# michalfratczak/habdec

Measured on AMD Instinct MI355X. Metric: IQ Msamples/s (batched 2.048 MS/s streams), higher is better.
Workload: dtype f32

## Files before the change

habdec_amd/csrc/dev_types.h:

```cpp
#pragma once
#include <stdint.h>
#ifndef __HIPCC__
#ifndef __host__
#define __host__
#define __device__
#endif
#endif

namespace hd {

constexpr int kFftBins = 4096;
constexpr uint32_t kVentLimit = 30000;
constexpr uint32_t kFirBatch = 256;

struct StreamCall {
    uint32_t n_in;
    uint32_t n1;
    uint32_t n2;
    uint32_t zero_hist1;
    uint32_t zero_hist2;
    uint32_t pend_before;
    uint32_t fft_fill;
    uint32_t fft_take;
    uint32_t fft_run;
    uint32_t fir_m;
    uint32_t fir_taps;
    uint32_t fir_zero_hist;
    uint32_t pend_after;
    uint32_t dc_remove;
    uint32_t clear_pending;
    uint32_t fir_taps_prev;
};
__host__ __device__ inline uint32_t sc_taps_prev(const StreamCall& c) { return c.fir_taps_prev & 0xFFFFu; }
__host__ __device__ inline uint32_t sc_head_n(const StreamCall& c) { return (c.fir_taps_prev >> 16) & 0x3FFFu; }
__host__ __device__ inline bool sc_head_prev(const StreamCall& c) { return (c.fir_taps_prev >> 30) & 1u; }
__host__ __device__ inline bool sc_head_save(const StreamCall& c) { return (c.fir_taps_prev >> 31) & 1u; }
__host__ __device__ inline uint32_t sc_pack_taps_prev(uint32_t taps_prev, uint32_t head_n, bool head_prev, bool head_save)
{ return (taps_prev & 0xFFFFu) | ((head_n & 0x3FFFu) << 16) | ((head_prev ? 1u : 0u) << 30) | ((head_save ? 1u : 0u) << 31); }


struct SymbolParams {
    uint32_t spb;
    uint32_t R;
    uint32_t min_held;
    uint32_t float_abs;
    uint32_t reset;
};

struct SymState {
    uint32_t base;
    uint32_t held;
    uint32_t cached;
    uint32_t run_pos;
    float    run_sum;
    uint32_t _pad[3];
};

struct BitsHeader {
    uint32_t nbits;
    uint32_t held_after;
    uint32_t nflips;
    uint32_t overflow;
    uint32_t uncached;
    uint32_t demod_ck[2];
    uint32_t demod_n;
// ... 15 lines not shown
```

habdec_amd/csrc/engine.cpp:

```cpp
#include <hip/hip_runtime.h>
#include <rocfft/rocfft.h>

#include <algorithm>
#include <atomic>
#include <chrono>
#include <cmath>
#include <cstdio>
#include <cstdlib>
#include <cstring>
#include <memory>
#include <condition_variable>
#include <mutex>
#include <thread>
#include <string>
#include <vector>

#include "../../include/habdec_amd.h"
#include "dev_types.h"
#include "host/afc_tracker.hpp"
#include "host/decim_plan.hpp"
#include "host/fir_design.hpp"
#include "host/iq_file_batch.hpp"
#include "host/text_stage.hpp"
#include "kernels/launch.h"
// ... 17 lines not shown
    size_t n = 0;
    hipError_t alloc(size_t count)
    {
        n = count;
        hipError_t e = hipMalloc(reinterpret_cast<void**>(&p), std::max<size_t>(count, 1) * sizeof(T));
        if (e == hipSuccess) e = hipMemset(p, 0, std::max<size_t>(count, 1) * sizeof(T));
        return e;
    }
    ~DevBuf() { if (p) (void)hipFree(p); }
};
template <typename T>
struct PinBuf {
    T* p = nullptr;
    T* dev = nullptr;
    size_t n = 0;
    hipError_t alloc(size_t count)
    {
        n = count;
        hipError_t e = hipHostMalloc(reinterpret_cast<void**>(&p), std::max<size_t>(count, 1) * sizeof(T), hipHostMallocMapped | hipHostMallocCoherent);
        if (e == hipSuccess) std::memset(p, 0, std::max<size_t>(count, 1) * sizeof(T));
        if (e == hipSuccess) e = hipHostGetDevicePointer(reinterpret_cast<void**>(&dev), p, 0);
        return e;
    }
    ~PinBuf() { if (p) (void)hipHostFree(p); }
};

struct StreamHost {
    double baud = 300;
    float lp_bw = 1500, lp_trans = 0.025f;
    bool dc = false;
    size_t stage_buf[2] = {0, 0};
    size_t pending = 0;
    size_t fft_fill = 0;
    bool have_spectrum = false;
    uint64_t spectra = 0;
    size_t fir_buf = 0;
    uint32_t fir_T_run = 0;
    uint32_t head_n = 0;
    uint64_t head_call = ~0ull;
    bool head_aside = false;
    hd::LowpassDesigner lp;
    bool taps_dirty = false;
    uint32_t held = 0, win_ub = 0, inflight_m = 0;
    bool sym_reset = true;
    hd::TextStage text;
    hd::AfcTracker afc;
    hd::SpectrumStats stats{};
    uint32_t last_n2 = 0, last_pend_before = 0, last_m = 0, last_nbits = 0, last_nflips = 0;
    uint64_t flip_list_full = 0;
    uint64_t bits_total = 0;
    int last_buf = 0;
    std::vector<uint32_t> last_words;
    uint32_t demod_ck[2] = {0, 0}, demod_ck_n = 0xFFFFFFFFu;
    uint64_t demod_ck_call = 0;
    uint64_t demod_ck_hash = 0xCBF29CE484222325ull;
    uint64_t demod_ck_calls = 0, demod_ck_unknown = 0;
};

}

struct hd_engine {
    hd_engine_config cfg{};
    double fs = 0, fsd = 0;
    std::vector<hd::DecimStage> stages;
    uint32_t S = 0, D = 1;
    uint32_t n1_cap = 0, n2_cap = 0;
    uint32_t taps_cap = 0, fir_hist_cap = 0;
// ... 274 lines not shown
    } else
        e->no_claim = true;
    if (e->stages.size() >= 1) {
        for (auto& h : e->hist1) HD_HIP(h.alloc((size_t)S * (e->stages[0].taps.size() - 1)));
        HD_HIP(e->stage_taps[0].alloc(e->stages[0].taps.size() + 1));
        HD_HIP(hipMemcpy(e->stage_taps[0].p, e->stages[0].taps.data(), e->stages[0].taps.size() * 4, hipMemcpyHostToDevice));
    }
    if (e->stages.size() == 2) {
        for (auto& h : e->hist2) HD_HIP(h.alloc((size_t)S * (e->stages[1].taps.size() - 1)));
        HD_HIP(e->stage_taps[1].alloc(e->stages[1].taps.size() + 1));
        HD_HIP(hipMemcpy(e->stage_taps[1].p, e->stages[1].taps.data(), e->stages[1].taps.size() * 4, hipMemcpyHostToDevice));
    }
    for (auto& b : e->fbuf) HD_HIP(b.alloc((size_t)S * e->fbuf_stride));
    HD_HIP(e->lp_taps.alloc((size_t)S * e->taps_cap));
    HD_HIP(e->demod.alloc((size_t)S * m_cap));
    if (cfg->keep_filtered) HD_HIP(e->filtered.alloc((size_t)S * m_cap));
    HD_HIP(e->tail.alloc((size_t)S * e->tail_cap));
    HD_HIP(e->weight.alloc((size_t)S * e->tail_cap));
    HD_HIP(e->flipmask.alloc((size_t)S * (e->tail_cap / 64)));
    HD_HIP(e->d_symstate.alloc(S));
    if (e->flips_cap) HD_HIP(e->flips_dbg.alloc((size_t)S * e->flips_cap));
    for (auto& c : e->carry) HD_HIP(c.alloc(S));
    e->head_cap = std::min<uint32_t>(e->taps_cap, 8192u);
    HD_HIP(e->fir_head.alloc((size_t)S * e->head_cap));
    HD_HIP(e->demod_ck_acc.alloc((size_t)2 * S));
    HD_HIP(e->d_sym.alloc(S));
    HD_HIP(e->h_sym.alloc(S));
    for (auto& sl : e->slot) {
        HD_HIP(sl.d_call.alloc(S));
        HD_HIP(sl.h_call.alloc(S));
        HD_HIP(sl.h_slots.alloc((size_t)S * e->slot_words));
    }
    if (cfg->enable_spectrum) {
        HD_HIP(e->fft_in.alloc((size_t)S * hd::kFftBins));
        HD_HIP(e->fft_raw.alloc((size_t)S * hd::kFftBins));
        HD_HIP(e->spec.alloc((size_t)S * hd::kFftBins));
        HD_HIP(e->power.alloc((size_t)S * hd::kFftBins));
        for (auto& sl : e->slot) HD_HIP(sl.h_stats.alloc(S));
        {
            std::vector<float2> tw(hd::kFftBins);
            for (size_t m = 0; m < hd::kFftBins; ++m) {
                const double a = 2.0 * 3.14159265358979323846264338327950288 * (double)m / (double)hd::kFftBins;
                tw[m] = make_float2((float)std::cos(a), (float)-std::sin(a));
            }
            HD_HIP(e->fft_tw.alloc(hd::kFftBins));
            HD_HIP(hipMemcpy(e->fft_tw.p, tw.data(), tw.size() * sizeof(float2), hipMemcpyHostToDevice));
            e->tail_fft = getenv("HD_ROCFFT") == nullptr;
            e->own_fft = e->tail_fft || getenv("HD_OWN_FFT") != nullptr;
        }
        std::call_once(g_rocfft_once, [] { rocfft_setup(); });
        const size_t len = hd::kFftBins;
        if (rocfft_plan_create(&e->fft_plan, rocfft_placement_notinplace, rocfft_transform_type_complex_forward,
                               rocfft_precision_single, 1, &len, S, nullptr) != rocfft_status_success)
            return fail(HD_ERR_DEVICE, "rocfft_plan_create failed");
        if (rocfft_execution_info_create(&e->fft_info) != rocfft_status_success)
            return fail(HD_ERR_DEVICE, "rocfft_execution_info_create failed");
        size_t wsz = 0;
        rocfft_plan_get_work_buffer_size(e->fft_plan, &wsz);
        if (wsz) {
            HD_HIP(e->fft_work.alloc(wsz));
            rocfft_execution_info_set_work_buffer(e->fft_info, e->fft_work.p, wsz);
        }
        rocfft_execution_info_set_stream(e->fft_info, e->qa);
    }
    if (e->fast && e->taps_cap >= hd_engine::kLpFftMinTaps && getenv("HD_NO_LP_FFT") == nullptr) {
        std::call_once(g_rocfft_once, [] { rocfft_setup(); });
        uint32_t N = 1;
        while (N < m_cap + e->taps_cap) N <<= 1;
        e->lpf_N[1] = N; e->lpf_N[0] = N / 2;
        size_t wmax = 0;
        for (int w = 0; w < 2; ++w) {
            const size_t len = e->lpf_N[w];
            if (rocfft_plan_create(&e->lpf_fwd[w], rocfft_placement_inplace, rocfft_transform_type_complex_forward, rocfft_precision_single, 1, &len, S, nullptr) != rocfft_status_success ||
                rocfft_plan_create(&e->lpf_inv[w], rocfft_placement_inplace, rocfft_transform_type_complex_inverse, rocfft_precision_single, 1, &len, S, nullptr) != rocfft_status_success)
                return fail(HD_ERR_DEVICE, "rocfft_plan_create (low-pass transforms) failed");
            for (rocfft_plan pl : {e->lpf_fwd[w], e->lpf_inv[w]}) { size_t wsz = 0; rocfft_plan_get_work_buffer_size(pl, &wsz); wmax = std::max(wmax, wsz); }
        }
        if (rocfft_execution_info_create(&e->lpf_info) != rocfft_status_success) return fail(HD_ERR_DEVICE, "rocfft_execution_info_create failed");
        if (wmax) { HD_HIP(e->lpf_workbuf.alloc(wmax)); rocfft_execution_info_set_work_buffer(e->lpf_info, e->lpf_workbuf.p, wmax); }
        HD_HIP(e->lpf_x.alloc((size_t)S * N));
        HD_HIP(e->lpf_k.alloc((size_t)S * N));
// ... 209 lines not shown
                    e->device_failed = true;
                    e->fail_cause = std::string(what) + " of stream " + std::to_string(s) + " does not carry its call's tag 200 ms after the completion event";
                    rc = fail(HD_ERR_DEVICE, e->fail_cause + ": the results of this engine are unreliable -- destroy the engine");
                    return;
                }
                if (spins > 64u) std::this_thread::yield();
            }
        };
        for (uint32_t s = 0; s < e->S && !e->device_failed && !timing_experiment; ++s) {
            await(&reinterpret_cast<const volatile hd::BitsHeader*>(sl.h_slots.p + (size_t)s * e->slot_words)->seq, "result slot", s);
            if (!e->device_failed && e->cfg.enable_spectrum && sl.h_stats.p && sl.h_call.p[s].fft_run)
                await(reinterpret_cast<const volatile uint32_t*>(&sl.h_stats.p[s].seq), "spectrum statistics", s);
        }
        std::atomic_thread_fence(std::memory_order_acquire);
    }
    if (e->ring_gave_up.p && e->ring_gave_up.p[0] && !e->device_failed) {
        e->device_failed = true;
        e->fail_cause = "k_stage1_cu (loader / consumer waves): a bounded wait ran out inside a launch (word " + std::to_string(e->ring_gave_up.p[0]) + ")";
    }
    if (e->device_failed && rc == HD_OK)
        rc = fail(HD_ERR_DEVICE, e->fail_cause + ": the results of this and of every later call of this engine are unreliable -- destroy the engine");
    if (e->device_failed) {
        e->last_timing.host_wait_us = std::chrono::duration<double, std::micro>(w1 - w0).count();
        e->last_timing.host_text_us = 0;
        return rc;
    }
    for (uint32_t s = 0; s < e->S; ++s) {
        StreamHost& st = e->st[s];
        const hd::StreamCall& c = sl.h_call.p[s];
        if (c.fft_run) {
            std::memcpy(&st.stats, &sl.h_stats.p[s], sizeof(st.stats));
            st.have_spectrum = true;
            ++st.spectra;
        }
        const bool past_batch_gate = c.fir_m || c.clear_pending;
        if (past_batch_gate && e->cfg.enable_spectrum) st.afc.step(st.have_spectrum, st.stats, hd::kFftBins, e->fsd);
        const uint32_t* slot = sl.h_slots.p + (size_t)s * e->slot_words;
        const hd::BitsHeader* hdr = reinterpret_cast<const hd::BitsHeader*>(slot);
        st.held = hdr->held_after;
        st.inflight_m -= c.fir_m;
        st.win_ub = hdr->uncached + st.inflight_m;
        st.last_nbits = hdr->nbits; st.last_nflips = hdr->nflips;
        st.bits_total += hdr->nbits;
        st.demod_ck[0] = hdr->demod_ck[0]; st.demod_ck[1] = hdr->demod_ck[1]; st.demod_ck_n = hdr->demod_n; st.demod_ck_call = e->delivered;
        if (hdr->demod_n != 0xFFFFFFFFu) {
            for (const uint32_t x : {hdr->demod_n, hdr->demod_ck[0], hdr->demod_ck[1]}) st.demod_ck_hash = (st.demod_ck_hash ^ x) * 0x100000001B3ull;
            ++st.demod_ck_calls;
        } else ++st.demod_ck_unknown;
        if (hdr->overflow & 1u) rc = fail(HD_ERR_CAPACITY, "symbol result slot overflow on stream " + std::to_string(s));
        if (hdr->overflow & 2u) ++st.flip_list_full;
        const uint32_t* words = slot + sizeof(hd::BitsHeader) / 4;
        st.last_words.assign(words, words + (hdr->nbits + 31) / 32);
        if (!c.fir_m) continue;
        if (hdr->nbits) st.text.framer.push_packed(words, hdr->nbits);
        const std::string chars = st.text.run(hdr->nbits != 0, [&](const hd::SentenceMatch& m) {
            ++e->sentences_ok;
            if (e->sentence_cb) { e->in_callback = true; e->sentence_cb(e->sentence_user, s, m.callsign.c_str(), m.data.c_str(), m.crc.c_str()); e->in_callback = false; }
        }, [&](const hd::SentenceMatch& m, bool ok) {
            if (e->match_cb) { e->in_callback = true; e->match_cb(e->match_user, s, m.callsign.c_str(), m.data.c_str(), m.crc.c_str(), ok ? 1 : 0); e->in_callback = false; }
        });
        if (!chars.empty() && e->chars_cb) { e->in_callback = true; e->chars_cb(e->chars_user, s, chars.data(), chars.size()); e->in_callback = false; }
    }
    e->last_timing.host_wait_us = std::chrono::duration<double, std::micro>(w1 - w0).count();
    e->last_timing.host_text_us = std::chrono::duration<double, std::micro>(std::chrono::steady_clock::now() - w1).count();
    return rc;
}
// ... 42 lines not shown
        const uint32_t n = n_per_stream ? n_per_stream[s] : n_uniform;
        if (n > e->cfg.max_chunk) return fail(HD_ERR_CAPACITY, "more samples than max_chunk");
        if (n % e->D) return fail(HD_ERR_INVALID, "sample count must be a multiple of the decimation factor (queue the remainder)");
        if (n && nst > 0 && n + 1 < T1) return fail(HD_ERR_UNSUPPORTED, "chunk shorter than the first stage's history (undefined in the reference)");
        if (n && nst > 1 && n / R1 + 1 < T2) return fail(HD_ERR_UNSUPPORTED, "chunk shorter than the second stage's history (undefined in the reference)");
    }
    bool tables_dirty = e->sym_dirty;
    for (uint32_t s = 0; s < S && !tables_dirty; ++s) tables_dirty = e->st[s].taps_dirty;
    if (tables_dirty) { if (int rc = flush_locked(e)) return rc; }

    hd_engine::CallSlot& sl = e->slot[e->calls % hd_engine::kSlots];
    while (sl.busy) {
        if (int rc = collect(e, e->slot[e->delivered % hd_engine::kSlots])) return rc;
        ++e->delivered;
    }

    uint32_t max_in = 0, min_in = 0xFFFFFFFFu, max_n1 = 0, max_n2 = 0, max_m = 0, max_taps = 0, max_new = 0, max_pend = 0;
    bool any_fft = false, any_dc = false, any_zero1 = false;
    uint64_t total_in = 0;
    for (uint32_t s = 0; s < S; ++s) {
        StreamHost& st = e->st[s];
        hd::StreamCall c{};
        const uint32_t n = n_per_stream ? n_per_stream[s] : n_uniform;
        c.n_in = n;
        c.n1 = n / R1;
        c.n2 = c.n1 / R2;
        if (n) {
            if (nst > 0) { const size_t want = (size_t)n + T1 + R1; if (st.stage_buf[0] < want) { st.stage_buf[0] = want; c.zero_hist1 = 1; } }
            if (nst > 1) { const size_t want = (size_t)c.n1 + T2 + R2; if (st.stage_buf[1] < want) { st.stage_buf[1] = want; c.zero_hist2 = 1; } }
        }
        c.dc_remove = st.dc && c.n2;
        c.pend_before = (uint32_t)st.pending;
        st.pending += c.n2;
        c.fft_fill = (uint32_t)st.fft_fill;
        if (e->cfg.enable_spectrum && n && st.fft_fill < (size_t)hd::kFftBins && c.n2) {
            c.fft_take = (uint32_t)std::min<size_t>(hd::kFftBins - st.fft_fill, c.n2);
            st.fft_fill += c.fft_take;
        }
        if (e->cfg.enable_spectrum && n && st.fft_fill >= (size_t)hd::kFftBins) { c.fft_run = 1; st.fft_fill = 0; any_fft = true; }
        const bool past_batch_gate = n && st.pending >= hd::kFirBatch;
        st.last_m = 0;
        if (past_batch_gate && !e->decode_enabled) { c.clear_pending = 1; st.pending = 0; }
        else if (past_batch_gate) {
            const uint32_t m = (uint32_t)(st.pending - st.pending % hd::kFirBatch);
            st.lp.batch = m;
            if (st.lp.design(cutoff_rel(e, st), st.lp_trans)) {
                st.taps_dirty = true;
                if (int rc = flush_locked(e)) return rc;
            }
            const uint32_t T = (uint32_t)st.lp.taps.size();
            if (!T) return fail(HD_ERR_UNSUPPORTED, "low-pass transition width leaves no taps (reference filters nothing then)");
            if (T > e->taps_cap) return fail(HD_ERR_CAPACITY, "low-pass tap count exceeds engine capacity");
            if (st.fir_buf < (size_t)m + T) { st.fir_buf = (size_t)m + T; c.fir_zero_hist = 1; }
            c.fir_m = m; c.fir_taps = T;
            c.fir_taps_prev = hd::sc_pack_taps_prev(st.fir_T_run ? st.fir_T_run : T, st.head_n, !st.head_aside && st.head_call + 1 == e->calls, false);
            st.fir_T_run = T;
            st.head_n = std::min<uint32_t>(m, std::min<uint32_t>(e->head_cap, 0x3FFFu)); st.head_call = e->calls; st.head_aside = false;
            st.pending -= m;
            st.last_m = m;
            max_m = std::max(max_m, m);
            max_taps = std::max(max_taps, T);
            const uint32_t pending_windows = st.sym_reset ? std::max(st.held, st.win_ub) : st.win_ub;
            max_new = std::max(max_new, pending_windows + m + 64u);
            st.inflight_m += m;
            st.win_ub += m;
        }
        if (!c.fir_m && st.head_n && !st.head_aside) {
            if (st.head_call + 1 == e->calls) c.fir_taps_prev = hd::sc_pack_taps_prev(0, st.head_n, false, true);
            else st.head_n = 0;
            st.head_aside = true;
        }
        c.pend_after = (uint32_t)st.pending;
// ... 1 lines not shown
        st.last_n2 = c.n2; st.last_pend_before = c.pend_before; st.last_buf = e->cur;
        sl.h_call.p[s] = c;
        max_in = std::max(max_in, n); min_in = std::min(min_in, n); max_n1 = std::max(max_n1, c.n1); max_n2 = std::max(max_n2, c.n2);
        any_dc |= c.dc_remove != 0;
        any_zero1 |= c.zero_hist1 != 0;
        total_in += n;
    }
    sl.total_in = total_in;
    sl.r1 = R1;
    sl.seq = (uint32_t)(e->calls + 1u);
    if (!sl.seq) sl.seq = 1u;
    hipStream_t qa = e->qa, qb = e->qb;
    hd::TailArgs ta{};
    const int tail_lanes = (S >= 2 * e->n_cus ? 64 : 256);
    const bool tail = nst == 2 && !any_dc && !e->no_tail && max_n2 <= e->tail_max_n2 &&
                      ((tail_lanes == 256 && max_n2 >= 512u && HDK(tail_layout, ta, tail_lanes, (int)R2, (int)T2, max_taps, e->max_R, e->min_R, e->tail_cap, max_pend, 64 * 1024, 4)) ||
                       HDK(tail_layout, ta, tail_lanes, (int)R2, (int)T2, max_taps, e->max_R, e->min_R, e->tail_cap, max_pend, 64 * 1024));
    const bool fuse = tail || (nst == 2 && !any_dc && !e->no_fuse && ((R2 == 2 && T2 == 69) || (R2 == 4 && T2 == 139)) &&
                      HDK(backend_lds_bytes, (int)T2, max_n1, max_n2, max_taps) <= 64 * 1024);
    hd::TailArgs ta_step{};
    const bool step = tail && e->cfg.pipeline && !e->one_stream && min_in == max_in && max_in && (R1 == 32 || R1 == 64) &&
                      HDK(step_lds_bytes, (int)R1, (int)T1) &&
                      HDK(tail_layout, ta_step, 64, (int)R2, (int)T2, max_taps, e->max_R, e->min_R, e->tail_cap, max_pend, HDK(step_lds_bytes, (int)R1, (int)T1));
    const int path = step ? 3 : tail ? 2 : fuse ? 1 : 0;
    if (e->last_fuse >= 0 && e->last_fuse != path) {
        if (const int r = run_pending_tail(e)) return r;
        HD_HIP(hipStreamSynchronize(qa)); HD_HIP(hipStreamSynchronize(qb));
    }
    e->last_fuse = path;
    e->last_timing.path = (uint32_t)path;
    if (path == 0 && e->own_fft && e->cfg.enable_spectrum && !any_dc && any_fft) {
        for (uint32_t s = 0; s < S; ++s) {
            hd::StreamCall& c = sl.h_call.p[s];
            if (c.fft_run == 1 && c.fft_fill == 0 && c.fft_take == (uint32_t)hd::kFftBins) { c.fft_take = 0; c.fft_run = 2; }
        }
    }
    const bool lean = fuse && !e->one_stream;
    const bool free_front = !fuse && nst == 2 && !e->one_stream;
    if (!lean && !free_front && e->calls >= 2 && !e->one_stream) HD_HIP(hipStreamWaitEvent(qa, e->slot[(e->calls - 2) % hd_engine::kSlots].ev_done, 0));
    sl.timed = e->timing_every && (e->calls % e->timing_every) == 0;
    sl.timed_step = sl.timed && step;
    if (sl.timed && !step) HD_HIP(hipEventRecord(sl.t0, qa));
    const bool host_params = tail && !step && e->one_stream && (!e->cfg.enable_spectrum || (e->tail_fft && !any_dc));
    if (lean || free_front) {
        if (e->sym_dirty && e->calls > e->delivered) { if (int rc = flush_locked(e)) return rc; }
    } else if (!host_params) {
        HDK(launch_fetch_params, e->qc, sl.h_call.dev, sl.d_call.p, S * sizeof(hd::StreamCall));
        if (!e->one_stream) { HD_HIP(hipEventRecord(sl.ev_params, e->qc)); HD_HIP(hipStreamWaitEvent(qa, sl.ev_params, 0)); }
    }
    for (uint32_t s = 0; s < S; ++s) {
        StreamHost& st = e->st[s];
        if (!st.taps_dirty) continue;
        HD_HIP(hipMemcpyAsync(e->lp_taps.p + (size_t)s * e->taps_cap, st.lp.taps.data(), st.lp.taps.size() * 4, hipMemcpyHostToDevice, qa));
        st.taps_dirty = false;
        e->lpf_k_stale = true;
    }
    if (e->sym_dirty) {
        uint32_t mr = 4;
        for (uint32_t s = 0; s < S; ++s) {
            e->h_sym.p[s] = symbol_params(e, e->st[s]);
            e->h_sym.p[s].reset = e->st[s].sym_reset ? 1u : 0u;
            mr = std::max(mr, e->h_sym.p[s].R);
        }
        e->max_R = mr;
        { uint32_t lo = mr; for (uint32_t s2 = 0; s2 < S; ++s2) lo = std::min(lo, std::max<uint32_t>(e->h_sym.p[s2].R, 4)); e->min_R = lo; }
        HD_HIP(hipMemcpyAsync(e->d_sym.p, e->h_sym.p, S * sizeof(hd::SymbolParams), hipMemcpyHostToDevice, qa));
        e->sym_dirty = false;
        for (uint32_t s = 0; s < S; ++s)
            if (e->st[s].sym_reset) { e->st[s].sym_reset = false; e->sym_dirty = true; }
    }
    const float2* iq = static_cast<const float2*>(d_iq);
    float2* fcur = e->fbuf[e->cur].p;
    float2* fnext = e->fbuf[(e->cur + 1) % 3].p;
    const hd::StreamCall* dcall = host_params ? sl.h_call.dev : sl.d_call.p;
    float2* d1 = (e->calls % 3 == 0) ? e->dec1.p : (e->calls % 3 == 1) ? e->dec1b.p : e->dec1c.p;
    const int hin = e->hist_cur, hout = e->hist_cur ^ 1;
    float2* feed = (e->cfg.enable_spectrum && !any_dc) ? e->fft_in.p : nullptr;
    const int cin = e->carry_cur, cout = e->carry_cur ^ 1;
    auto fill_tail = [&](hd::TailArgs& t) {
        t.dec1 = d1; t.dec1_stride = e->n1_cap; t.hist2_in = e->hist2[hin].p; t.hist2_out = e->hist2[hout].p; t.taps2 = e->stage_taps[1].p;
        t.fbuf = fcur; t.fbuf_next = fnext; t.fbuf_stride = e->fbuf_stride; t.fir_hist_cap = e->fir_hist_cap;
        t.lp_taps = e->lp_taps.p; t.taps_stride = e->taps_cap; t.demod = e->demod.p; t.demod_stride = e->demod.n / S;
        t.filtered = e->cfg.keep_filtered ? e->filtered.p : nullptr; t.carry_in = e->carry[cin].p; t.carry_out = e->carry[cout].p;
        t.call = dcall; t.fft_in = feed; t.head_buf = e->fir_head.p; t.fbuf_prev = e->fbuf[(e->cur + 2) % 3].p; t.head_cap = e->head_cap;
        t.n_streams = S;
        t.ring = e->tail.p; t.ring_cap = e->tail_cap; t.sym = e->d_symstate.p; t.flipmask = e->flipmask.p; t.wsum = e->weight.p;
        t.sp = e->d_sym.p; t.slots = sl.h_slots.dev; t.slot_words = e->slot_words; t.seq = sl.seq;
        t.flips_dbg = e->flips_cap ? e->flips_dbg.p : nullptr; t.flips_cap = e->flips_cap;
        const bool in_tail = e->tail_fft && e->cfg.enable_spectrum && feed;
        t.fft_tw = in_tail ? e->fft_tw.p : nullptr; t.spec = e->spec.p; t.power = e->power.p; t.stats = sl.h_stats.dev; t.rate = e->fsd; t.bins_sep = e->bins_sep;
    };
    auto make_claim = [&](uint32_t lin_wgs ,
                          uint32_t run_len_cu = 0 ) {
        hd::StepClaim claim{};
        const uint32_t ntiles = run_len_cu ? HDK(ring_tiles, (int)R1, (int)T1, max_in) : (max_n1 + 63) / 64, n_xcd = e->n_cus / 32u, run_len = run_len_cu ? run_len_cu : e->step_run >= 2 ? e->step_run : 4u;
        const uint64_t runs = (uint64_t)S * ntiles / run_len;
        const bool shape_ok = run_len_cu ? (HDK(stage1_cu_supported, (int)R1, (int)T1) && max_in % 2048u == 0) : ((R1 == 32 || R1 == 64) && max_n1 % 64 == 0);
        if (!e->no_claim && (nst == 2 || (run_len_cu && nst == 1)) && shape_ok && min_in == max_in && max_in && !any_zero1 && n_xcd && e->n_cus % 32u == 0 && n_xcd <= 16 &&
            ntiles && (ntiles % run_len == 0 || (run_len_cu && R1 >= 32 && ((uint64_t)S * ntiles) % run_len == 0)) && runs % n_xcd == 0 && (uint64_t)S * ntiles < (1ull << 32) && (uint64_t)ntiles * S >= 4ull * lin_wgs) {
            claim.ctr = e->step_ctr.p + (size_t)(e->step_launches & 1u) * 16 * 32;
            claim.ctr_next = e->step_ctr.p + (size_t)((e->step_launches & 1u) ^ 1u) * 16 * 32;
            claim.n_xcd = n_xcd; claim.runs_per_xcd = (uint32_t)(runs / n_xcd); claim.run_len = run_len;
            if (run_len_cu && R1 >= 32 && e->ring_short_pct) {
                const uint32_t tpx = claim.runs_per_xcd * run_len, whole = (uint32_t)((uint64_t)tpx * (100u - e->ring_short_pct) / 100u) / run_len;
                claim.tiles_per_xcd = tpx; claim.short_from = whole; claim.runs_per_xcd = whole + (tpx - whole * run_len);
            }
            ++e->step_launches;
        }
        return claim;
    };
    auto pick_ring_run = [&](const uint32_t ntiles) -> uint32_t {
        const uint32_t n_xcd = e->n_cus / 32u ? e->n_cus / 32u : 1u, want = R1 >= 32 ? 4u : 8u;
        auto ok = [&](uint32_t r) { return r >= 2u && r <= ntiles && (R1 >= 32 ? ((uint64_t)S * ntiles) % r == 0 : ntiles % r == 0) && ((uint64_t)S * ntiles / r) % n_xcd == 0; };
        if (e->ring_run >= 2 && ok(e->ring_run)) return e->ring_run;
        for (uint32_t d = 0; d <= 8u; ++d) {
            if (ok(want + d)) return want + d;
            if (d && d < want && ok(want - d)) return want - d;
        }
        return 2u;
    };
    if (step) {
        const uint32_t ring_nt = HDK(ring_tiles, (int)R1, (int)T1, max_in), ring_run0 = pick_ring_run(ring_nt), n_xcd0 = e->n_cus / 32u;
        const bool runs_ok = ring_nt && n_xcd0 && ring_run0 >= 2u && ((uint64_t)S * ring_nt) % ring_run0 == 0 && ((uint64_t)S * ring_nt / ring_run0) % n_xcd0 == 0;
// ... 353 lines not shown
{ if (check_stream(e, s)) return 0; std::lock_guard<std::recursive_mutex> l(e->mtx); return copy_out(e->st[s].text.stream, buf, cap); }
size_t hd_stream_last_sentence(hd_engine* e, uint32_t s, char* buf, size_t cap)
{ if (check_stream(e, s)) return 0; std::lock_guard<std::recursive_mutex> l(e->mtx); return copy_out(e->st[s].text.last_sentence, buf, cap); }
size_t hd_stream_take_sentences(hd_engine* e, uint32_t s, char* buf, size_t cap)
{ if (check_stream(e, s)) return 0; std::lock_guard<std::recursive_mutex> l(e->mtx); return take_out(e->st[s].text.ok_log, buf, cap); }
size_t hd_stream_take_matches(hd_engine* e, uint32_t s, char* buf, size_t cap)
{ if (check_stream(e, s)) return 0; std::lock_guard<std::recursive_mutex> l(e->mtx); return take_out(e->st[s].text.match_log, buf, cap); }
size_t hd_stream_take_chars(hd_engine* e, uint32_t s, char* buf, size_t cap)
{ if (check_stream(e, s)) return 0; std::lock_guard<std::recursive_mutex> l(e->mtx); return take_out(e->st[s].text.char_log, buf, cap); }

int hd_stream_afc(hd_engine* e, uint32_t s, hd_afc_info* out)
{
    if (int r = check_stream(e, s)) return r;
    if (!out) return fail(HD_ERR_INVALID, "null argument");
    std::lock_guard<std::recursive_mutex> l(e->mtx);
    const StreamHost& st = e->st[s];
    out->frequency_correction = st.afc.correction; out->shift_hz = st.afc.shift_hz;
    out->noise_floor = st.afc.noise_floor; out->noise_variance = st.afc.noise_sigma;
    out->peak_left = st.afc.gui_left; out->peak_right = st.afc.gui_right; out->spectra = st.spectra;
    return HD_OK;
}

static size_t fetch(hd_engine* e, const void* dev, size_t count, size_t elem, void* host, size_t cap)
{
    if (e->in_callback) { fail(HD_ERR_INVALID, "data getters cannot be called from a sentence / character callback (text getters can)"); return 0; }
    (void)flush_locked(e);
    const size_t n = std::min(count, cap);
    if (!n || !host) return count;
    if (hipSetDevice(e->cfg.device) != hipSuccess) return 0;
    if (hipMemcpy(host, dev, n * elem, hipMemcpyDeviceToHost) != hipSuccess) return 0;
    return count;
}

size_t hd_stream_spectrum(hd_engine* e, uint32_t s, float* iq, size_t cap)
{
    if (check_stream(e, s)) return 0;
    std::lock_guard<std::recursive_mutex> l(e->mtx);
    if (!e->cfg.enable_spectrum || !e->st[s].have_spectrum) return 0;
    return fetch(e, e->spec.p + (size_t)s * hd::kFftBins, hd::kFftBins, sizeof(float2), iq, cap);
}
size_t hd_stream_power(hd_engine* e, uint32_t s, float* p, size_t cap)
{
    if (check_stream(e, s)) return 0;
    std::lock_guard<std::recursive_mutex> l(e->mtx);
    if (!e->cfg.enable_spectrum || !e->st[s].have_spectrum) return 0;
    return fetch(e, e->power.p + (size_t)s * hd::kFftBins, hd::kFftBins, sizeof(float), p, cap);
}
size_t hd_stream_demodulated(hd_engine* e, uint32_t s, float* v, size_t cap)
{
    if (check_stream(e, s)) return 0;
    std::lock_guard<std::recursive_mutex> l(e->mtx);
    return fetch(e, e->demod.p + (size_t)s * (e->demod.n / e->S), e->st[s].last_m, sizeof(float), v, cap);
}
size_t hd_stream_decimated(hd_engine* e, uint32_t s, float* iq, size_t cap)
{
    if (check_stream(e, s)) return 0;
    std::lock_guard<std::recursive_mutex> l(e->mtx);
    const StreamHost& st = e->st[s];
    const float2* src = e->fbuf[st.last_buf].p + (size_t)s * e->fbuf_stride + e->fir_hist_cap + st.last_pend_before;
    return fetch(e, src, st.last_n2, sizeof(float2), iq, cap);
}
size_t hd_stream_filtered(hd_engine* e, uint32_t s, float* iq, size_t cap)
{
    if (check_stream(e, s)) return 0;
    std::lock_guard<std::recursive_mutex> l(e->mtx);
    if (!e->cfg.keep_filtered) return 0;
    return fetch(e, e->filtered.p + (size_t)s * (e->demod.n / e->S), e->st[s].last_m, sizeof(float2), iq, cap);
}
size_t hd_stream_bits(hd_engine* e, uint32_t s, uint8_t* bits, size_t cap)
{
    if (check_stream(e, s)) return 0;
    std::lock_guard<std::recursive_mutex> l(e->mtx);
    const StreamHost& st = e->st[s];
    for (uint32_t i = 0; i < st.last_nbits && i < cap; ++i) bits[i] = (st.last_words[i >> 5] >> (i & 31)) & 1u;
    return st.last_nbits;
}
size_t hd_stream_flips(hd_engine* e, uint32_t s, uint32_t* flips, size_t cap)
{
    if (check_stream(e, s)) return 0;
// ... 54 lines not shown
```

habdec_amd/csrc/kernels/launch.h:

```cpp
#pragma once
#include <hip/hip_runtime.h>
#include <stddef.h>
#include <stdint.h>

#include "../dev_types.h"

namespace hd {

struct DemodCarry {
    float re, im;
    uint32_t primed;
    uint32_t _pad;
};

struct StepClaim {
    unsigned int* ctr = nullptr;
    unsigned int* ctr_next = nullptr;
    uint32_t n_xcd = 0, runs_per_xcd = 0, run_len = 0;
    uint32_t short_from = 0xFFFFFFFFu, tiles_per_xcd = 0;
};

struct TailArgs {
    const float2* dec1; size_t dec1_stride;
    const float2* hist2_in; float2* hist2_out; const float* taps2;
    float2* fbuf; float2* fbuf_next; size_t fbuf_stride; uint32_t fir_hist_cap;
    const float* lp_taps; uint32_t taps_stride;
    float* demod; size_t demod_stride; float2* filtered;
    const DemodCarry* carry_in; DemodCarry* carry_out;
    const StreamCall* call; float2* fft_in;
    float2* head_buf ; const float2* fbuf_prev ; uint32_t head_cap, n_streams;
    float* ring; uint32_t ring_cap; SymState* sym; unsigned long long* flipmask; float* wsum; const SymbolParams* sp;
    uint32_t* slots; uint32_t slot_words; uint32_t* flips_dbg; uint32_t flips_cap;
    uint32_t seq;
    const float2* fft_tw; float2* spec; float* power; SpectrumStatsDev* stats; double rate; int bins_sep;
    uint32_t pend_max, f_off, v_off, ws_off, words_off, tp_off, h2_off, flips_off, fl_cap, strips_off, dyn_off, lds_bytes;
    uint32_t op;
};

constexpr uint32_t kStepLdsBytes = 20480;

void launch_spectrum_commit(hipStream_t st, uint32_t n_streams, const float2* raw, float2* spec, float* power,
                            SpectrumStatsDev* stats, const StreamCall* call, double rate, int bins_sep,
                            uint32_t seq );
void launch_spectrum_wave(hipStream_t st, uint32_t n_streams, const float2* fft_in, const float2* tw4096, float2* spec, float* power,
                          SpectrumStatsDev* stats, const StreamCall* call, double rate, int bins_sep, uint32_t seq,
                          const float2* chunk = nullptr ,
                          size_t chunk_stride = 0, uint32_t fir_hist_cap = 0);

namespace exact {
#include "launch_decls.inc"
}
namespace fast {
#include "launch_decls.inc"
}

}
```

habdec_amd/csrc/kernels/spectrum_wave.h:

```cpp
#pragma once
#include <hip/hip_runtime.h>

#include "launch.h"
#include "sym_common.h"

namespace hd {

namespace specwave {

__device__ static constexpr float kW64[2][32] = {
#include "fft64_tw.inc"
};

constexpr int xpos(int k) { return 8 * (k & 7) + (k >> 3); }

__device__ __forceinline__ void fft8(f32x2 (&v)[8])
{
    constexpr float r = 0.70710678118654752440f;
    const f32x2 a0 = v[0] + v[4], a1 = v[0] - v[4], a2 = v[2] + v[6], a3 = v[2] - v[6];
    const f32x2 a4 = v[1] + v[5], a5 = v[1] - v[5], a6 = v[3] + v[7], a7 = v[3] - v[7];
    const f32x2 a3r = (f32x2){a3.y, -a3.x}, a7r = (f32x2){a7.y, -a7.x};
    const f32x2 b0 = a0 + a2, b2 = a0 - a2, b1 = a1 + a3r, b3 = a1 - a3r;
    const f32x2 b4 = a4 + a6, b6 = a4 - a6, b5 = a5 + a7r, b7 = a5 - a7r;
    const f32x2 t5 = (f32x2){(b5.x + b5.y) * r, (b5.y - b5.x) * r};
// ... 34 lines not shown
        fft8(v);
#pragma unroll
        for (int k2 = 0; k2 < 8; ++k2) a[8 * k1 + k2] = v[k2];
    }
    __builtin_amdgcn_sched_barrier(0);
}

__device__ __forceinline__ void pin64(f32x2 (&a)[64])
{
#pragma unroll
    for (int i = 0; i < 64; ++i) asm volatile("" : "+v"(a[i]));
}

__device__ __forceinline__ double wave_sum(double v)
{
    for (int off = 32; off > 0; off >>= 1) v += __shfl_down(v, off, 64);
    return __shfl(v, 0, 64);
}

__device__ __forceinline__ void wave_argmax(float& v, int& idx)
{
    for (int off = 32; off > 0; off >>= 1) {
        const float ov = __shfl_down(v, off, 64);
        const int oi = __shfl_down(idx, off, 64);
        if (ov > v || (ov == v && oi < idx)) { v = ov; idx = oi; }
    }
    v = __shfl(v, 0, 64); idx = __shfl(idx, 0, 64);
}

}

constexpr uint32_t kSpecWaveLds = 64 * 65 * 4;

__device__ __forceinline__ void spectrum_wave_body(const float2* __restrict__ x, const float2* __restrict__ tw4096, float2* __restrict__ spec,
                                                   float* __restrict__ power, SpectrumStatsDev* __restrict__ stats, const uint32_t s, const double rate,
                                                   const int bins_sep, float* __restrict__ plane, const uint32_t seq)
{
    const uint32_t l = threadIdx.x & 63u;
    f32x2 a[64];
#pragma unroll
    for (int g = 0; g < 64; g += 8) {
        const float2* xg = x + 64 * g;
        asm volatile("" : "+s"(xg));
#pragma unroll
        for (int u = 0; u < 8; ++u) { const float2 v = xg[64 * u + l]; a[g + u] = (f32x2){v.x, v.y}; }
    }
    specwave::fft64(a);
#pragma unroll
    for (int g = 0; g < 64; g += 16) {
        __builtin_amdgcn_sched_barrier(0);
        float2 w[16];
#pragma unroll
        for (int u = 0; u < 16; ++u) w[u] = tw4096[(l * (uint32_t)specwave::xpos(g + u)) & (kFftBins - 1)];
#pragma unroll
        for (int u = 0; u < 16; ++u) {
            const f32x2 v = a[g + u];
            a[g + u] = (f32x2){v.x * w[u].x - v.y * w[u].y, v.x * w[u].y + v.y * w[u].x};
        }
    }
    __builtin_amdgcn_sched_barrier(0);
#pragma unroll
    for (int k1 = 0; k1 < 64; ++k1) plane[k1 * 65 + l] = a[specwave::xpos(k1)].x;
    __builtin_amdgcn_s_waitcnt(0xC07F);
    __builtin_amdgcn_wave_barrier();
#pragma unroll
    for (int n2 = 0; n2 < 64; ++n2) a[n2].x = plane[l * 65 + n2];
    __builtin_amdgcn_s_waitcnt(0xC07F);
    __builtin_amdgcn_wave_barrier();
#pragma unroll
    for (int k1 = 0; k1 < 64; ++k1) plane[k1 * 65 + l] = a[specwave::xpos(k1)].y;
    __builtin_amdgcn_s_waitcnt(0xC07F);
    __builtin_amdgcn_wave_barrier();
#pragma unroll
    for (int n2 = 0; n2 < 64; ++n2) a[n2].y = plane[l * 65 + n2];
    specwave::pin64(a);
    specwave::fft64(a);
    specwave::pin64(a);
    float2* so = spec + (size_t)s * kFftBins;
    float* po = power + (size_t)s * kFftBins;
    int mybad = 0;
    double lsum = 0.0;
#define HD_SW_P(j_) a[specwave::xpos(((j_) + 32) & 63)].x
    float2* sg = so;
    float* pg = po;
#pragma unroll
    for (int j = 0; j < 64; ++j) {
        if ((j & 7) == 0) {
            __builtin_amdgcn_sched_barrier(0);
            sg = so + 64 * j; pg = po + 64 * j;
            asm volatile("" : "+s"(sg), "+s"(pg));
        }
        const int k2 = (j + 32) & 63;
        const f32x2 v = a[specwave::xpos(k2)];
        sg[l + 64 * (j & 7)] = make_float2(v.x, v.y);
        float q = (v.x * v.x + v.y * v.y) / (float)kFftBins;
        q = q * q;
        q = (float)((double)q / rate);
        q = 10.0f * log10f(q);
        if (v.x != v.x || v.y != v.y || isinf(v.x) || isinf(v.y) || q != q || isinf(q)) mybad = 1;
        HD_SW_P(j) = q;
        pg[l + 64 * (j & 7)] = q;
        lsum += (double)q;
    }
    const bool bad = __builtin_amdgcn_ballot_w64(mybad != 0) != 0ull;
    const double mean = specwave::wave_sum(lsum) / (double)kFftBins;
    double lvar = 0.0;
    float bv = -__builtin_huge_valf();
    int bi = kFftBins;
#pragma unroll
    for (int j = 0; j < 64; ++j) {
        const float pj = HD_SW_P(j);
        const double d = (double)pj - mean;
        lvar += d * d;
        if (pj > bv) { bv = pj; bi = (int)l + 64 * j; }
    }
    const double sigma = sqrt(specwave::wave_sum(lvar) / (double)kFftBins);
    specwave::wave_argmax(bv, bi);
    const int p1 = bi;
    const float p1v = bv;
    const int lo = max(p1 - 2 * bins_sep, 0), hi = min(p1 + 2 * bins_sep, (int)kFftBins);
    const float floor0 = __shfl(HD_SW_P(0), 0, 64);
    float cv = -__builtin_huge_valf();
    int ci = kFftBins;
#pragma unroll
    for (int j = 0; j < 64; ++j) {
        const int i = (int)l + 64 * j;
        const float pj = HD_SW_P(j);
        if (i >= lo && i < hi && pj > floor0 && abs(i - p1) > bins_sep / 2 && pj > cv) { cv = pj; ci = i; }
    }
    specwave::wave_argmax(cv, ci);
    if (l == 0) {
        int pa = p1, pb = 0;
        float av = p1v, bvv = floor0;
        if (ci < (int)kFftBins) { pb = ci; bvv = cv; }
        if (pb < pa) { const int ti = pa; pa = pb; pb = ti; const float tv = av; av = bvv; bvv = tv; }
        SpectrumStatsDev o;
        o.valid = bad ? 0 : 1;
// ... 11 lines not shown
```

habdec_amd/csrc/kernels/spectrum_wave.hip:

```cpp
#include <hip/hip_runtime.h>

#include "spectrum_wave.h"

namespace hd {

__global__ __launch_bounds__(64) __attribute__((amdgpu_waves_per_eu(2, 2))) void k_spectrum_wave(const float2* __restrict__ fft_in, const float2* __restrict__ tw4096, float2* __restrict__ spec,
                                                        float* __restrict__ power, SpectrumStatsDev* __restrict__ stats,
                                                        const StreamCall* __restrict__ call, double rate, int bins_sep, const uint32_t seq,
                                                        const float2* __restrict__ chunk, const size_t chunk_stride, const uint32_t fir_hist_cap)
{
    __shared__ float plane[64 * 65];
    const uint32_t s = blockIdx.x;
    const uint32_t run = call[s].fft_run;
    if (!run) return;
    const float2* x = run == 2u ? chunk + (size_t)s * chunk_stride + fir_hist_cap + call[s].pend_before : fft_in + (size_t)s * kFftBins;
    spectrum_wave_body(x, tw4096, spec, power, stats, s, rate, bins_sep, plane, seq);
}

void launch_spectrum_wave(hipStream_t st, uint32_t n_streams, const float2* fft_in, const float2* tw4096, float2* spec, float* power,
                          SpectrumStatsDev* stats, const StreamCall* call, double rate, int bins_sep, uint32_t seq, const float2* chunk, size_t chunk_stride, uint32_t fir_hist_cap)
{
    hipLaunchKernelGGL(k_spectrum_wave, dim3(n_streams), dim3(64), 0, st, fft_in, tw4096, spec, power, stats, call, rate, bins_sep, seq, chunk, chunk_stride, fir_hist_cap);
}

}
```

habdec_amd/csrc/kernels/tail_body.h:

```cpp
#pragma once
#include <hip/hip_runtime.h>

#include "arith.h"
#include "exact_math.h"
#include "launch.h"
#include "sym_common.h"
#include "spectrum_wave.h"

namespace hd {
namespace HD_ARITH_NS {

constexpr uint32_t kTailHdrBytes = 64;
constexpr uint32_t kTailStrip = 512;

typedef float f32x4 __attribute__((ext_vector_type(4)));
typedef const float __attribute__((address_space(4)))* cfloat_ptr;
__device__ __forceinline__ cfloat_ptr as_const(const float* p) { return (cfloat_ptr)(uintptr_t)p; }

#define HD_TB_TAP4(A_, B_, C_, D_, k_)                                                        \
    {                                                                                         \
        HD_FIR_ARITH                                                                          \
        const f32x2 p0_ = (A_) * (k_), p1_ = (B_) * (k_), p2_ = (C_) * (k_), p3_ = (D_) * (k_); \
        a0 = a0 + p0_; a1 = a1 + p1_; a2 = a2 + p2_; a3 = a3 + p3_;                           \
    }
// ... 822 lines not shown
        if (nbits & 31) outw[nbits >> 5] = curw;
        if (a.flips_dbg)
            for (uint32_t r = 0; r < nfl && r < a.flips_cap; ++r) a.flips_dbg[(size_t)s * a.flips_cap + r] = flips[r];
        const uint32_t last = nfl ? flips[nfl - 1] : 0u;
        st.run_pos = st.base + max(nfl ? last : carried_to, frontier);
        st.run_sum = __builtin_bit_cast(float, sh[3]);
        st.cached = pend;
        st.base += last;
        st.held = h - last;
        a.sym[s] = st;
        hdr->nbits = nbits; hdr->held_after = st.held; hdr->nflips = nfl; hdr->overflow = overflow; hdr->uncached = end - st.cached;
    }
    TSTAMP(11);
    };
    second_half();
    {
#pragma unroll
        for (int o = 32; o >= 1; o >>= 1) { ck0 += (uint32_t)__shfl_xor((int)ck0, o, 64); ck1 += (uint32_t)__shfl_xor((int)ck1, o, 64); }
        if constexpr (NT == 64) {
            if (tid == 0) { hdr->demod_ck[0] = ck0; hdr->demod_ck[1] = ck1; hdr->demod_n = m; }
        } else {
            tb_sync<NT>();
            if (tid == 0) { sh[5] = 0; sh[6] = 0; }
            tb_sync<NT>();
            if (lane == 0) { atomicAdd(&sh[5], ck0); atomicAdd(&sh[6], ck1); }
            tb_sync<NT>();
            if (tid == 0) { hdr->demod_ck[0] = sh[5]; hdr->demod_ck[1] = sh[6]; hdr->demod_n = m; }
        }
    }
    if (a.fft_tw && c.fft_run) {
        __threadfence_block();
        tb_sync<NT>();
        if (wave == 0)
            spectrum_wave_body(a.fft_in + (size_t)s * kFftBins, a.fft_tw, a.spec, a.power, a.stats, s, a.rate, a.bins_sep, reinterpret_cast<float*>(lds + kTailHdrBytes), a.seq);
    }
    asm volatile("s_waitcnt vmcnt(0)" ::: "memory");
#ifdef HD_RING_FAULT
    if (tid == 0 && g_tail_fault_armed && atomicCAS(&g_tail_fault_fired, 0u, 1u) == 0u) return;
#endif
    if (tid == 0) __hip_atomic_store(&hdr->seq, a.seq, __ATOMIC_RELAXED, __HIP_MEMORY_SCOPE_SYSTEM);
    TSTAMP_WRITE();
}

}
}
```

Before: 504,400.

## Defer spectrum and power writes to on-demand getter, double-buffer FFT input

The per-call spectrum FFT no longer writes the 4096-bin complex spectrum and power arrays. It computes only the stats the AFC needs. The FFT input buffer is double-buffered so the last completed window stays available, and a single-block kernel recomputes spectrum and power lazily when a host getter asks for them. This removes global-memory stores from the hot tail kernel, at the cost of extra buffer memory and a synchronous launch inside the getters.

```diff
diff --git a/habdec_amd/csrc/dev_types.h b/habdec_amd/csrc/dev_types.h
--- a/habdec_amd/csrc/dev_types.h
+++ b/habdec_amd/csrc/dev_types.h
@@ -31,6 +31,8 @@
     uint32_t clear_pending;
     uint32_t fir_taps_prev;
 };
+__host__ __device__ inline uint32_t sc_fft_row(const StreamCall& c) { return c.fft_fill & ~(uint32_t)(kFftBins - 1); }
+
 __host__ __device__ inline uint32_t sc_taps_prev(const StreamCall& c) { return c.fir_taps_prev & 0xFFFFu; }
 __host__ __device__ inline uint32_t sc_head_n(const StreamCall& c) { return (c.fir_taps_prev >> 16) & 0x3FFFu; }
 __host__ __device__ inline bool sc_head_prev(const StreamCall& c) { return (c.fir_taps_prev >> 30) & 1u; }
diff --git a/habdec_amd/csrc/engine.cpp b/habdec_amd/csrc/engine.cpp
--- a/habdec_amd/csrc/engine.cpp
+++ b/habdec_amd/csrc/engine.cpp
@@ -73,7 +73,11 @@
     size_t stage_buf[2] = {0, 0};
     size_t pending = 0;
     size_t fft_fill = 0;
+    uint32_t fft_half = 0;
     bool have_spectrum = false;
+    bool spec_lazy = false;
+    bool spec_made = false;
+    uint32_t spec_row = 0;
     uint64_t spectra = 0;
     size_t fir_buf = 0;
     uint32_t fir_T_run = 0;
@@ -414,7 +418,9 @@
         HD_HIP(sl.h_slots.alloc((size_t)S * e->slot_words));
     }
     if (cfg->enable_spectrum) {
-        HD_HIP(e->fft_in.alloc((size_t)S * hd::kFftBins));
+        e->tail_fft = getenv("HD_ROCFFT") == nullptr;
+        e->own_fft = e->tail_fft || getenv("HD_OWN_FFT") != nullptr;
+        HD_HIP(e->fft_in.alloc((size_t)(e->own_fft ? 2 : 1) * S * hd::kFftBins));
         HD_HIP(e->fft_raw.alloc((size_t)S * hd::kFftBins));
         HD_HIP(e->spec.alloc((size_t)S * hd::kFftBins));
         HD_HIP(e->power.alloc((size_t)S * hd::kFftBins));
@@ -427,8 +433,6 @@
             }
             HD_HIP(e->fft_tw.alloc(hd::kFftBins));
             HD_HIP(hipMemcpy(e->fft_tw.p, tw.data(), tw.size() * sizeof(float2), hipMemcpyHostToDevice));
-            e->tail_fft = getenv("HD_ROCFFT") == nullptr;
-            e->own_fft = e->tail_fft || getenv("HD_OWN_FFT") != nullptr;
         }
         std::call_once(g_rocfft_once, [] { rocfft_setup(); });
         const size_t len = hd::kFftBins;
@@ -704,6 +708,9 @@
             std::memcpy(&st.stats, &sl.h_stats.p[s], sizeof(st.stats));
             st.have_spectrum = true;
             ++st.spectra;
+            st.spec_lazy = e->own_fft && c.fft_run == 1;
+            st.spec_made = false;
+            st.spec_row = hd::sc_fft_row(c);
         }
         const bool past_batch_gate = c.fir_m || c.clear_pending;
         if (past_batch_gate && e->cfg.enable_spectrum) st.afc.step(st.have_spectrum, st.stats, hd::kFftBins, e->fsd);
@@ -812,12 +819,15 @@
         c.dc_remove = st.dc && c.n2;
         c.pend_before = (uint32_t)st.pending;
         st.pending += c.n2;
-        c.fft_fill = (uint32_t)st.fft_fill;
+        c.fft_fill = (uint32_t)st.fft_fill + st.fft_half * S * (uint32_t)hd::kFftBins;
         if (e->cfg.enable_spectrum && n && st.fft_fill < (size_t)hd::kFftBins && c.n2) {
             c.fft_take = (uint32_t)std::min<size_t>(hd::kFftBins - st.fft_fill, c.n2);
             st.fft_fill += c.fft_take;
         }
-        if (e->cfg.enable_spectrum && n && st.fft_fill >= (size_t)hd::kFftBins) { c.fft_run = 1; st.fft_fill = 0; any_fft = true; }
+        if (e->cfg.enable_spectrum && n && st.fft_fill >= (size_t)hd::kFftBins) {
+            c.fft_run = 1; st.fft_fill = 0; any_fft = true;
+            if (e->own_fft) st.fft_half ^= 1u;
+        }
         const bool past_batch_gate = n && st.pending >= hd::kFirBatch;
         st.last_m = 0;
         if (past_batch_gate && !e->decode_enabled) { c.clear_pending = 1; st.pending = 0; }
@@ -885,7 +895,7 @@
     if (path == 0 && e->own_fft && e->cfg.enable_spectrum && !any_dc && any_fft) {
         for (uint32_t s = 0; s < S; ++s) {
             hd::StreamCall& c = sl.h_call.p[s];
-            if (c.fft_run == 1 && c.fft_fill == 0 && c.fft_take == (uint32_t)hd::kFftBins) { c.fft_take = 0; c.fft_run = 2; }
+            if (c.fft_run == 1 && (c.fft_fill & (hd::kFftBins - 1)) == 0 && c.fft_take == (uint32_t)hd::kFftBins) { c.fft_take = 0; c.fft_run = 2; }
         }
     }
     const bool lean = fuse && !e->one_stream;
@@ -941,7 +951,7 @@
         t.sp = e->d_sym.p; t.slots = sl.h_slots.dev; t.slot_words = e->slot_words; t.seq = sl.seq;
         t.flips_dbg = e->flips_cap ? e->flips_dbg.p : nullptr; t.flips_cap = e->flips_cap;
         const bool in_tail = e->tail_fft && e->cfg.enable_spectrum && feed;
-        t.fft_tw = in_tail ? e->fft_tw.p : nullptr; t.spec = e->spec.p; t.power = e->power.p; t.stats = sl.h_stats.dev; t.rate = e->fsd; t.bins_sep = e->bins_sep;
+        t.fft_tw = in_tail ? e->fft_tw.p : nullptr; t.stats = sl.h_stats.dev; t.rate = e->fsd; t.bins_sep = e->bins_sep;
     };
     auto make_claim = [&](uint32_t lin_wgs ,
                           uint32_t run_len_cu = 0 ) {
@@ -1361,19 +1371,32 @@
     return count;
 }
 
+static size_t fetch_spectrum(hd_engine* e, uint32_t s, const void* dev, size_t elem, void* host, size_t cap)
+{
+    if (e->in_callback) { fail(HD_ERR_INVALID, "data getters cannot be called from a sentence / character callback (text getters can)"); return 0; }
+    (void)flush_locked(e);
+    StreamHost& st = e->st[s];
+    if (st.spec_lazy && !st.spec_made && host && cap && !e->device_failed) {
+        if (hipSetDevice(e->cfg.device) != hipSuccess) return 0;
+        hd::launch_spectrum_one(e->qa, s, e->fft_in.p + (size_t)s * hd::kFftBins + st.spec_row, e->fft_tw.p, e->spec.p, e->power.p, e->fsd, e->bins_sep);
+        if (hipGetLastError() != hipSuccess || hipStreamSynchronize(e->qa) != hipSuccess) return 0;
+        st.spec_made = true;
+    }
+    return fetch(e, dev, hd::kFftBins, elem, host, cap);
+}
 size_t hd_stream_spectrum(hd_engine* e, uint32_t s, float* iq, size_t cap)
 {
     if (check_stream(e, s)) return 0;
     std::lock_guard<std::recursive_mutex> l(e->mtx);
     if (!e->cfg.enable_spectrum || !e->st[s].have_spectrum) return 0;
-    return fetch(e, e->spec.p + (size_t)s * hd::kFftBins, hd::kFftBins, sizeof(float2), iq, cap);
+    return fetch_spectrum(e, s, e->spec.p + (size_t)s * hd::kFftBins, sizeof(float2), iq, cap);
 }
 size_t hd_stream_power(hd_engine* e, uint32_t s, float* p, size_t cap)
 {
     if (check_stream(e, s)) return 0;
     std::lock_guard<std::recursive_mutex> l(e->mtx);
     if (!e->cfg.enable_spectrum || !e->st[s].have_spectrum) return 0;
-    return fetch(e, e->power.p + (size_t)s * hd::kFftBins, hd::kFftBins, sizeof(float), p, cap);
+    return fetch_spectrum(e, s, e->power.p + (size_t)s * hd::kFftBins, sizeof(float), p, cap);
 }
 size_t hd_stream_demodulated(hd_engine* e, uint32_t s, float* v, size_t cap)
 {
diff --git a/habdec_amd/csrc/kernels/launch.h b/habdec_amd/csrc/kernels/launch.h
--- a/habdec_amd/csrc/kernels/launch.h
+++ b/habdec_amd/csrc/kernels/launch.h
@@ -32,7 +32,7 @@
     float* ring; uint32_t ring_cap; SymState* sym; unsigned long long* flipmask; float* wsum; const SymbolParams* sp;
     uint32_t* slots; uint32_t slot_words; uint32_t* flips_dbg; uint32_t flips_cap;
     uint32_t seq;
-    const float2* fft_tw; float2* spec; float* power; SpectrumStatsDev* stats; double rate; int bins_sep;
+    const float2* fft_tw; SpectrumStatsDev* stats; double rate; int bins_sep;
     uint32_t pend_max, f_off, v_off, ws_off, words_off, tp_off, h2_off, flips_off, fl_cap, strips_off, dyn_off, lds_bytes;
     uint32_t op;
 };
@@ -46,6 +46,7 @@
                           SpectrumStatsDev* stats, const StreamCall* call, double rate, int bins_sep, uint32_t seq,
                           const float2* chunk = nullptr ,
                           size_t chunk_stride = 0, uint32_t fir_hist_cap = 0);
+void launch_spectrum_one(hipStream_t st, uint32_t s, const float2* x, const float2* tw4096, float2* spec, float* power, double rate, int bins_sep);
 
 namespace exact {
 #include "launch_decls.inc"
diff --git a/habdec_amd/csrc/kernels/spectrum_wave.h b/habdec_amd/csrc/kernels/spectrum_wave.h
--- a/habdec_amd/csrc/kernels/spectrum_wave.h
+++ b/habdec_amd/csrc/kernels/spectrum_wave.h
@@ -90,6 +90,7 @@
 
 constexpr uint32_t kSpecWaveLds = 64 * 65 * 4;
 
+template <bool kSpec, bool kStats>
 __device__ __forceinline__ void spectrum_wave_body(const float2* __restrict__ x, const float2* __restrict__ tw4096, float2* __restrict__ spec,
                                                    float* __restrict__ power, SpectrumStatsDev* __restrict__ stats, const uint32_t s, const double rate,
                                                    const int bins_sep, float* __restrict__ plane, const uint32_t seq)
@@ -134,8 +135,9 @@
     specwave::pin64(a);
     specwave::fft64(a);
     specwave::pin64(a);
-    float2* so = spec + (size_t)s * kFftBins;
-    float* po = power + (size_t)s * kFftBins;
+    float2* so = nullptr;
+    float* po = nullptr;
+    if constexpr (kSpec) { so = spec + (size_t)s * kFftBins; po = power + (size_t)s * kFftBins; }
     int mybad = 0;
     double lsum = 0.0;
 #define HD_SW_P(j_) a[specwave::xpos(((j_) + 32) & 63)].x
@@ -145,22 +147,25 @@
     for (int j = 0; j < 64; ++j) {
         if ((j & 7) == 0) {
             __builtin_amdgcn_sched_barrier(0);
-            sg = so + 64 * j; pg = po + 64 * j;
-            asm volatile("" : "+s"(sg), "+s"(pg));
+            if constexpr (kSpec) {
+                sg = so + 64 * j; pg = po + 64 * j;
+                asm volatile("" : "+s"(sg), "+s"(pg));
+            }
         }
         const int k2 = (j + 32) & 63;
         const f32x2 v = a[specwave::xpos(k2)];
-        sg[l + 64 * (j & 7)] = make_float2(v.x, v.y);
+        if constexpr (kSpec) sg[l + 64 * (j & 7)] = make_float2(v.x, v.y);
         float q = (v.x * v.x + v.y * v.y) / (float)kFftBins;
         q = q * q;
         q = (float)((double)q / rate);
         q = 10.0f * log10f(q);
         if (v.x != v.x || v.y != v.y || isinf(v.x) || isinf(v.y) || q != q || isinf(q)) mybad = 1;
         HD_SW_P(j) = q;
-        pg[l + 64 * (j & 7)] = q;
+        if constexpr (kSpec) pg[l + 64 * (j & 7)] = q;
         lsum += (double)q;
     }
     const bool bad = __builtin_amdgcn_ballot_w64(mybad != 0) != 0ull;
+    if constexpr (!kStats) return;
     const double mean = specwave::wave_sum(lsum) / (double)kFftBins;
     double lvar = 0.0;
     float bv = -__builtin_huge_valf();
diff --git a/habdec_amd/csrc/kernels/spectrum_wave.hip b/habdec_amd/csrc/kernels/spectrum_wave.hip
--- a/habdec_amd/csrc/kernels/spectrum_wave.hip
+++ b/habdec_amd/csrc/kernels/spectrum_wave.hip
@@ -13,8 +13,15 @@
     const uint32_t s = blockIdx.x;
     const uint32_t run = call[s].fft_run;
     if (!run) return;
-    const float2* x = run == 2u ? chunk + (size_t)s * chunk_stride + fir_hist_cap + call[s].pend_before : fft_in + (size_t)s * kFftBins;
-    spectrum_wave_body(x, tw4096, spec, power, stats, s, rate, bins_sep, plane, seq);
+    if (run == 2u) spectrum_wave_body<true, true>(chunk + (size_t)s * chunk_stride + fir_hist_cap + call[s].pend_before, tw4096, spec, power, stats, s, rate, bins_sep, plane, seq);
+    else spectrum_wave_body<false, true>(fft_in + (size_t)s * kFftBins + sc_fft_row(call[s]), tw4096, spec, power, stats, s, rate, bins_sep, plane, seq);
+}
+
+__global__ __launch_bounds__(64) void k_spectrum_one(const float2* __restrict__ x, const float2* __restrict__ tw4096, float2* __restrict__ spec, float* __restrict__ power,
+                                                     const uint32_t s, const double rate, const int bins_sep)
+{
+    __shared__ float plane[64 * 65];
+    spectrum_wave_body<true, false>(x, tw4096, spec, power, nullptr, s, rate, bins_sep, plane, 0u);
 }
 
 void launch_spectrum_wave(hipStream_t st, uint32_t n_streams, const float2* fft_in, const float2* tw4096, float2* spec, float* power,
@@ -23,4 +30,9 @@
     hipLaunchKernelGGL(k_spectrum_wave, dim3(n_streams), dim3(64), 0, st, fft_in, tw4096, spec, power, stats, call, rate, bins_sep, seq, chunk, chunk_stride, fir_hist_cap);
 }
 
+void launch_spectrum_one(hipStream_t st, uint32_t s, const float2* x, const float2* tw4096, float2* spec, float* power, double rate, int bins_sep)
+{
+    hipLaunchKernelGGL(k_spectrum_one, dim3(1), dim3(64), 0, st, x, tw4096, spec, power, s, rate, bins_sep);
 }
+
+}
diff --git a/habdec_amd/csrc/kernels/tail_body.h b/habdec_amd/csrc/kernels/tail_body.h
--- a/habdec_amd/csrc/kernels/tail_body.h
+++ b/habdec_amd/csrc/kernels/tail_body.h
@@ -878,7 +878,8 @@
         __threadfence_block();
         tb_sync<NT>();
         if (wave == 0)
-            spectrum_wave_body(a.fft_in + (size_t)s * kFftBins, a.fft_tw, a.spec, a.power, a.stats, s, a.rate, a.bins_sep, reinterpret_cast<float*>(lds + kTailHdrBytes), a.seq);
+            spectrum_wave_body<false, true>(a.fft_in + (size_t)s * kFftBins + sc_fft_row(c), a.fft_tw, nullptr, nullptr, a.stats, s, a.rate, a.bins_sep,
+                                            reinterpret_cast<float*>(lds + kTailHdrBytes), a.seq);
     }
     asm volatile("s_waitcnt vmcnt(0)" ::: "memory");
 #ifdef HD_RING_FAULT
```

New measurement: 511,200, median of 6. 1.01x the previous value.
